# alexrenz/AdaPM

Measured on AMD Instinct MI355X. Metric: pull_push_ops_per_s, higher is better.
Workload: dtype fp32; 1 GPU; model=kge_complex_dim512, entities=10000000, relations=1000, dim=512, neg_samples=16, global_batch=16384, triples=90000000, parallelism=ps-async-dp1, fused_step=True, warmup_extra_steps=400

## Files before the change

### adapm_amd/csrc/core.cpp

```cpp
#include <torch/extension.h>
#include <ATen/Parallel.h>

#include <algorithm>
#include <atomic>
#include <condition_variable>
#include <cstring>
#include <limits>
#include <deque>
#include <map>
#include <queue>
#include <tuple>
#include <memory>
#include <mutex>
#include <random>
#include <thread>
#include <chrono>
#include <unordered_map>
#include <unordered_set>
#include <cstdio>
#include <vector>

#include "common.h"
#include "kernels.h"
#include "ops.h"
#include "ustream.h"

#ifdef ADAPM_WITH_HIP
#include <c10/hip/HIPStream.h>
#include <ATen/core/CachingHostAllocator.h>
#include <ATen/hip/impl/HIPStreamMasqueradingAsCUDA.h>
#endif

extern "C" {
int adapm_host_arena_alloc(long long floats, int want_device_visible, void** host_ptr,
                           void** dev_ptr);
void adapm_host_arena_free(void* host_ptr, int was_device_visible);
}

namespace adapm {

namespace py = pybind11;

static void* current_stream(const torch::Device& dev) {
#ifdef ADAPM_WITH_HIP
  if (dev.is_cuda()) return (void*)c10::hip::getCurrentHIPStream(dev.index()).stream();
#endif
  return nullptr;
}

static void check_step_lanes(const char* name, const char* what, int64_t lanes) {
  TORCH_CHECK(lanes <= STEP_MAX_LANES, name, ": ", what, " = ", lanes,
              " exceeds the GPU step kernels' limit of ", STEP_MAX_LANES);
}


struct Slab {
  torch::Tensor buf;
  float* data = nullptr;
  int64_t capacity = 0;
  int64_t bump = 0;
  std::unordered_map<int32_t, std::vector<int64_t>> freelists;
  std::mutex mu;
  std::atomic<int64_t> in_use{0};
  bool is_cuda = false;
  void* host_raw = nullptr;
  float* host_host = nullptr;
  float* host_dev = nullptr;
  int64_t host_capacity = 0;
  int64_t host_bump = 0;
  std::unordered_map<int32_t, std::vector<int64_t>> host_freelists;
  std::atomic<int64_t> host_in_use{0};

  static int32_t padded(int32_t len) { return (len + 3) & ~3; }

  void init(int64_t cap, const torch::Device& dev) {
    capacity = cap;
    is_cuda = dev.is_cuda();
    buf = torch::zeros({cap}, torch::TensorOptions().dtype(torch::kFloat32).device(dev));
    data = buf.data_ptr<float>();
  }

  void init_host(int64_t cap) {
    void *hp = nullptr, *dp = nullptr;
    int rc = adapm_host_arena_alloc(cap, is_cuda ? 1 : 0, &hp, &dp);
    if (rc != 0) throw std::runtime_error("host-spill arena allocation failed");
    host_raw = hp;
    host_host = (float*)hp;
    host_dev = (float*)dp;
    host_capacity = cap;
  }
  ~Slab() { adapm_host_arena_free(host_raw, is_cuda ? 1 : 0); }

  SlabBases bases() const { return SlabBases{data, is_cuda ? host_dev : host_host}; }

  int64_t try_alloc_device(int32_t len) {
    int32_t p = padded(len);
    std::lock_guard<std::mutex> g(mu);
    auto it = freelists.find(p);
    if (it != freelists.end() && !it->second.empty()) {
      int64_t off = it->second.back();
      it->second.pop_back();
      in_use += p;
      return off;
    }
    if (bump + p <= capacity) {
      int64_t off = bump;
      bump += p;
      in_use += p;
      return off;
    }
    return -1;
  }

  int64_t alloc(int32_t len) {
    int32_t p = padded(len);
    std::lock_guard<std::mutex> g(mu);
    auto it = freelists.find(p);
    if (it != freelists.end() && !it->second.empty()) {
      int64_t off = it->second.back();
      it->second.pop_back();
      in_use += p;
      return off;
    }
    if (bump + p <= capacity) {
      int64_t off = bump;
      bump += p;
      in_use += p;
      return off;
    }
    if (host_capacity > 0) {
      auto hit = host_freelists.find(p);
      if (hit != host_freelists.end() && !hit->second.empty()) {
        int64_t off = hit->second.back();
        hit->second.pop_back();
        host_in_use += p;
        return off | SPILL_BIT;
// ... 48 lines not shown
struct RespRec {
  int dest = 0;
  int64_t code = 0, key = 0, f0 = 0, f1 = 0, f2 = 0;
  int64_t slab_off = -1;
  int32_t len = 0;
  bool free_after = false;
  torch::Tensor payload;
  std::vector<Key> keys;
  std::vector<int64_t> aux;
  std::vector<int64_t> aux2;
  std::vector<int64_t> slab_offs;
};

struct IntentReq {
  int wid;
  Clock start, end;
  std::vector<Key> keys;
};

struct ChannelState {
  std::mutex mu;
  std::deque<IntentReq> intent_queue;
  std::vector<IntentReq> future_intents;
  struct IntentExpiry {
    Clock end;
    int wid;
    std::shared_ptr<std::vector<Key>> keys;
    bool operator>(const IntentExpiry& o) const { return end > o.end; }
  };
  std::priority_queue<IntentExpiry, std::vector<IntentExpiry>, std::greater<>> intent_expiry;
  std::unordered_set<Key> replicas;
  std::unordered_map<Key, uint64_t> holders;
  std::deque<OutRec> out_queue;
  std::vector<RespRec> responses;
  std::unordered_map<Key, uint32_t> reloc_ctr;
  std::unordered_map<Key, int64_t> reloc_round;
  std::atomic<int64_t> rounds{0};
  int64_t idle_streak = 0;
  std::atomic<int64_t> idle2_events{0};
};


class UniformStream {
 public:
  UniformStream(int64_t lo, int64_t hi, const std::string& device)
      : lo_(lo), hi_(hi), dev_(device) {
    TORCH_CHECK(supported(lo, hi), "UniformStream: [", lo, ", ", hi,
                ") is not a range of numpy's 32-bit bounded draw");
    excl_ = (uint32_t)((uint64_t)hi - (uint64_t)lo);
    thr_ = (uint32_t)((0x100000000ull - excl_) % excl_);
    state_ = torch::zeros({USTREAM_STATE_WORDS},
                          torch::TensorOptions().dtype(torch::kInt64).device(dev_));
  }

  static bool supported(int64_t lo, int64_t hi) {
    if (hi <= lo || lo == std::numeric_limits<int64_t>::min()) return false;
    uint64_t span = (uint64_t)hi - (uint64_t)lo;
    return span >= 2 && span <= 0xFFFFFFFFull;
  }

  void import_state(uint64_t state_hi, uint64_t state_lo, uint64_t inc_hi, uint64_t inc_lo,
                    uint64_t has_uint32, uint64_t uinteger) {
    auto h = torch::empty({USTREAM_STATE_WORDS}, torch::kInt64);
    uint64_t* p = reinterpret_cast<uint64_t*>(h.data_ptr<int64_t>());
    p[0] = state_hi, p[1] = state_lo, p[2] = inc_hi, p[3] = inc_lo;
    p[4] = has_uint32 ? 1 : 0, p[5] = uinteger & 0xFFFFFFFFull;
    ustream_build_table(p);
    std::lock_guard<std::mutex> g(mu_);
    adopt(current_stream(dev_));
    state_.copy_(h);
  }

  std::vector<uint64_t> export_state() {
    torch::Tensor h;
    {
      std::lock_guard<std::mutex> g(mu_);
      adopt(current_stream(dev_));
      h = state_.slice(0, 0, USTREAM_GEN_WORDS).cpu();
    }
    const uint64_t* p = reinterpret_cast<const uint64_t*>(h.data_ptr<int64_t>());
    return std::vector<uint64_t>(p, p + USTREAM_GEN_WORDS);
  }

  torch::Tensor draw(int64_t n, int64_t slack = -1) {
    TORCH_CHECK(n >= 0, "UniformStream.draw: n must be >= 0");
    auto opt = torch::TensorOptions().dtype(torch::kInt64).device(dev_);
    auto out = torch::empty({n}, opt);
    if (n == 0) return out;
    if (slack < 0) {
      double p = (double)thr_ / 4294967296.0;
      double w0 = (double)n / (1.0 - p);
      slack = (int64_t)std::ceil(w0 - (double)n + 8.0 * std::sqrt(w0 * p) / (1.0 - p)) + 16;
    }
    const int64_t words = n + slack;
    std::lock_guard<std::mutex> g(mu_);
    void* st = current_stream(dev_);
    adopt(st);
    auto tmp = torch::empty({ustream_tmp_words(words)}, opt);
    uint64_t* sp = reinterpret_cast<uint64_t*>(state_.data_ptr<int64_t>());
    if (dev_.is_cuda()) {
#ifdef ADAPM_WITH_HIP
      uniform_draw_gpu(sp, lo_, excl_, thr_, n, words, out.data_ptr<int64_t>(),
                       tmp.data_ptr<int64_t>(), st);
#else
      TORCH_CHECK(false, "UniformStream: built without HIP");
#endif
    } else {
      uniform_draw_cpu(sp, lo_, excl_, thr_, n, words, out.data_ptr<int64_t>(),
                       tmp.data_ptr<int64_t>());
    }
    return out;
  }

  int64_t lo() const { return lo_; }
  int64_t hi() const { return hi_; }
  const torch::Device& device() const { return dev_; }

 private:
  void adopt(void* st) {
#ifdef ADAPM_WITH_HIP
    if (dev_.is_cuda() && have_owner_ && st != owner_) hipStreamSynchronize((hipStream_t)owner_);
#endif
    owner_ = st;
    have_owner_ = true;
  }

  int64_t lo_, hi_;
  uint32_t excl_ = 0, thr_ = 0;
  torch::Device dev_;
  torch::Tensor state_;
  std::mutex mu_;
  void* owner_ = nullptr;
  bool have_owner_ = false;
};


class Server {
 public:
  Server(int64_t num_keys, torch::Tensor lens, int rank, int world, int num_channels,
         int num_workers, std::string device, double capacity_factor, int techniques,
         bool location_caches, int64_t device_cap_floats = 0, int64_t host_spill_floats = 0,
         double sync_threshold = 0.0)
      : num_keys_(num_keys),
        rank_(rank),
        world_(world),
        nch_(num_channels),
        techniques_(techniques),
        use_loc_cache_(location_caches),
        sync_threshold_(sync_threshold),
        dev_(device) {
    TORCH_CHECK((nch_ & (nch_ - 1)) == 0, "num_channels must be a power of 2");
    {
      int hw = (int)std::thread::hardware_concurrency();
      int nt = std::max(1, std::min(hw / std::max(1, world_) - 2, 31));
      if (const char* e = getenv("ADAPM_PASS_THREADS")) nt = std::max(1, atoi(e));
      pass_pool_.want_threads = nt;
    }
    log2ch_ = 0;
    while ((1 << log2ch_) < nch_) log2ch_++;

    lens = lens.to(torch::kInt32).contiguous();
    if (lens.numel() == 1) {
      uniform_len_ = lens.item<int32_t>();
    } else {
      TORCH_CHECK(lens.numel() == num_keys_, "value_lengths must have num_keys entries");
      uniform_len_ = -1;
      lens_.assign(lens.data_ptr<int32_t>(), lens.data_ptr<int32_t>() + num_keys_);
    }

    meta_ = std::vector<std::atomic<int64_t>>(num_keys_);
    version_ = std::vector<std::atomic<uint32_t>>(num_keys_);
    for (int64_t i = 0; i < num_keys_; ++i) {
      meta_[i].store(0, std::memory_order_relaxed);
      version_[i].store(0, std::memory_order_relaxed);
    }
    sync_loc_.assign(num_keys_, -1);
    if (use_loc_cache_) loc_cache_.assign(num_keys_, -1);
    int64_t n_managed = (num_keys_ + world_ - 1) / world_;
    owner_of_.assign(n_managed, rank_);
    mgr_reloc_ctr_.assign(n_managed, 0);

    int64_t owned_floats = 0;
    for (Key k = rank_; k < num_keys_; k += world_) owned_floats += Slab::padded(len_of(k));
    int64_t cap = (int64_t)((double)owned_floats * capacity_factor) + (1 << 20);
    if (device_cap_floats > 0) cap = device_cap_floats;
    slab_.init(cap, dev_);
    if (host_spill_floats > 0) {
      slab_.init_host(host_spill_floats);
      heat_.reset(new std::atomic<uint32_t>[num_keys_]);
      for (Key k = 0; k < num_keys_; ++k) heat_[k].store(0, std::memory_order_relaxed);
    }
    if (owned_floats > cap) layout_identity_.store(false);
    for (Key k = rank_; k < num_keys_; k += world_) {
      int32_t l = len_of(k);
      meta_[k] = mpack(slab_.alloc(l), F_PRESENT | F_OWNER);
    }

    intent_cnt_.reset(new std::atomic<uint16_t>[num_keys_]);
    for (Key k = 0; k < num_keys_; ++k) intent_cnt_[k].store(0, std::memory_order_relaxed);
    channels_ = std::vector<ChannelState>(nch_);
    clocks_ = std::vector<std::atomic<Clock>>(std::max(1, num_workers));
    for (auto& c : clocks_) c = 0;
    locks_ = std::make_unique<std::mutex[]>(N_STRIPES);
  }


  static constexpr int64_t MSPILL = 16;
  static constexpr int64_t MFLAGS = F_PRESENT | F_OWNER | F_STUB | F_UPDATED | F_HASREP;
  static inline int64_t mpack(int64_t loc, int64_t flags) {
    if (loc < 0) return flags;
    return ((loc & ~SPILL_BIT) << 6) | ((loc & SPILL_BIT) ? MSPILL : 0) | flags;
  }
  static inline uint8_t mflags(int64_t m) { return (uint8_t)(m & MFLAGS); }
  static inline int64_t mloc(int64_t m) {
    return (int64_t)((uint64_t)m >> 6) | ((m & MSPILL) ? SPILL_BIT : 0);
  }

  inline bool on_default_stream() const {
#ifdef ADAPM_WITH_HIP
    if (dev_.is_cuda())
      return c10::hip::getCurrentHIPStream(dev_.index()) ==
             c10::hip::getDefaultHIPStream(dev_.index());
#endif
    return true;
  }

  inline int32_t len_of(Key k) const { return uniform_len_ >= 0 ? uniform_len_ : lens_[k]; }
  inline int manager_of(Key k) const { return (int)(k % world_); }
  inline int channel_of(Key k) const {
    if (nch_ == 1) return 0;
    return (int)(((uint32_t)((uint64_t)k * 2654435769ULL)) >> (32 - log2ch_));
  }
  inline std::mutex& stripe(Key k) { return locks_[(size_t)k % N_STRIPES]; }

  int directions(Key k) {
    if (meta_[k].load(std::memory_order_acquire) & F_OWNER) return rank_;
    if (manager_of(k) == rank_) return owner_of_[k / world_];
    if (use_loc_cache_) {
      int c = loc_cache_[k];
      if (c >= 0) return c;
    }
    return manager_of(k);
  }

  struct InflightGuard {
    Server* s;
    explicit InflightGuard(Server* sv) : s(sv) {
      for (;;) {
        s->inflight_.fetch_add(1, std::memory_order_acquire);
        if (!s->migrating_.load(std::memory_order_acquire)) break;
        s->inflight_.fetch_sub(1, std::memory_order_release);
        std::this_thread::yield();
      }
    }
    ~InflightGuard() { s->inflight_.fetch_sub(1, std::memory_order_release); }
  };

  void quiesce() {
    while (inflight_.load(std::memory_order_acquire) != 0) std::this_thread::yield();
  }


  struct HostBatch {
    std::vector<int64_t> src, dst;
    std::vector<int32_t> len;
    void add(int64_t s, int64_t d, int32_t l) {
      src.push_back(s);
      dst.push_back(d);
      len.push_back(l);
    }
    size_t size() const { return src.size(); }
  };

  struct PassPool {
    struct Task {
      const std::function<void(int64_t, int64_t)>* fn = nullptr;
      int64_t n = 0;
      std::atomic<int64_t>* next = nullptr;
      std::atomic<int>* done = nullptr;
      uint64_t gen = 0;
    };
    std::vector<std::thread> threads;
    std::mutex run_mu_;
    std::mutex mu;
    std::condition_variable cv;
    Task task;
    uint64_t gen = 0;
// ... 1907 lines not shown
      if (!it->second->fail.empty()) failed_tickets_[ts] = std::move(it->second->fail);
      tickets_.erase(it);
      tickets_cv_.notify_all();
    }
  }

  void fail_ticket(int64_t ts, int cnt, const char* why) {
    std::lock_guard<std::mutex> g(tickets_mu_);
    auto it = tickets_.find(ts);
    if (it == tickets_.end()) return;
    Ticket& t = *it->second;
    t.received += cnt;
    if (t.fail.empty()) t.fail = why;
    if (t.received >= t.expected) {
      failed_tickets_[ts] = std::move(t.fail);
      tickets_.erase(it);
      tickets_cv_.notify_all();
    }
  }

  void fail(std::string reason) {
    {
      std::lock_guard<std::mutex> g(tickets_mu_);
      failed_reason_ = std::move(reason);
      failed_flag_.store(true, std::memory_order_relaxed);
      tickets_.clear();
    }
    tickets_cv_.notify_all();
    rounds_cv_.notify_all();
  }
  std::string failed_reason() {
    std::lock_guard<std::mutex> g(tickets_mu_);
    return failed_reason_;
  }

  void sync_finish(int ch, bool globally_idle = false) {
    if (globally_idle) {
      std::lock_guard<std::mutex> g(channels_[ch].mu);
      if (!channels_[ch].responses.empty()) globally_idle = false;
      for (const auto& r : channels_[ch].out_queue) {
        bool data = (r.payload.defined() && r.payload.numel() > 0) ||
                    r.code == M_PUSH_REQ || r.code == M_SET_REQ || r.code == M_PUSH_REQ_BULK;
        if (data) {
          globally_idle = false;
          break;
        }
      }
    }
    {
      std::lock_guard<std::mutex> g(rounds_mu_);
      ChannelState& C = channels_[ch];
      C.rounds++;
      if (globally_idle) {
        if (++C.idle_streak >= 2) C.idle2_events++;
      } else {
        C.idle_streak = 0;
      }
    }
    rounds_cv_.notify_all();
  }

  py::dict debug_pending() {
    py::dict d;
    {
      std::lock_guard<std::mutex> g(tickets_mu_);
      d["tickets"] = tickets_.size();
    }
    py::list outq, respq, rounds;
    for (auto& C : channels_) {
      std::lock_guard<std::mutex> g(C.mu);
      outq.append(C.out_queue.size());
      respq.append(C.responses.size());
      rounds.append(C.rounds.load());
    }
    d["out_queues"] = outq;
    d["responses"] = respq;
    d["rounds"] = rounds;
    return d;
  }


  bool fused_plain_ok(void* st) {
    if (clocks_.size() != 1 || fused_multi_stream_) return false;
    if (!fused_marks_.defined()) {
      if (getenv("ADAPM_FUSED_ATOMIC")) {
        fused_multi_stream_ = true;
        return false;
      }
      fused_marks_ = torch::zeros({rowmark_words(num_keys_)},
                                  torch::TensorOptions().dtype(torch::kInt32).device(dev_));
      if (getenv("ADAPM_FUSED_STATS"))
        fused_shared_stat_ =
            torch::zeros({1}, torch::TensorOptions().dtype(torch::kInt64).device(dev_));
      fused_marks_stream_ = st;
      return true;
    }
    if (st == fused_marks_stream_) return true;
#ifdef ADAPM_WITH_HIP
    hipStreamSynchronize((hipStream_t)fused_marks_stream_);
#endif
    fused_multi_stream_ = true;
    return false;
  }

  void check_fused_identity(const char* name, int64_t D) {
    TORCH_CHECK(world_ == 1, name, " requires a single rank (all keys local)");
    TORCH_CHECK(uniform_len_ == 2 * D, name, ": store rows must be [emb|accum] = 2D");
    TORCH_CHECK(layout_identity_.load(), name, " requires the identity layout");
    TORCH_CHECK(dev_.is_cuda(), name, " is the GPU fast path");
  }

  void count_fused_ops(int64_t keys) {
    stat_pull_keys_ += keys;
    stat_pull_local_ += keys;
    stat_push_keys_ += keys;
    stat_push_local_ += keys;
    stat_pulls_ += 1;
    stat_pushes_ += 1;
  }

  struct StagedKeys {
    torch::Tensor dev;
    std::vector<const int64_t*> ptr;
  };
  StagedKeys stage_keys(const char* name, std::initializer_list<const torch::Tensor*> parts) {
    int64_t total = 0;
    for (auto* t : parts) {
      check_keys(*t);
      total += t->numel();
    }
    auto blob = torch::empty(
        {total}, torch::TensorOptions().dtype(torch::kInt64).pinned_memory(true));
    int64_t* dst = blob.data_ptr<int64_t>();
    const uint64_t lim = (uint64_t)num_keys_;
    uint64_t bad = 0;
    for (auto* t : parts) {
      const int64_t* kp = t->data_ptr<int64_t>();
      const int64_t n = t->numel();
      for (int64_t i = 0; i < n; ++i) {
        int64_t k = kp[i];
        dst[i] = k;
        bad |= ((uint64_t)k >= lim);
      }
      dst += n;
    }
    if (bad)
      for (auto* t : parts) check_key_range(*t);
    StagedKeys sk;
    sk.dev = torch::empty({total}, torch::TensorOptions().dtype(torch::kInt64).device(dev_));
#ifdef ADAPM_WITH_HIP
    auto stream = c10::hip::getCurrentHIPStreamMasqueradingAsCUDA(dev_.index());
    TORCH_CHECK(copy_keys_gpu(sk.dev.data_ptr<int64_t>(), blob.data_ptr<int64_t>(), total,
                              (void*)stream.stream()),
                name, ": the pinned key staging buffer is not visible to the device");
    at::getHostAllocator(at::kCUDA)->record_event(
        blob.data_ptr(), blob.storage().data_ptr().get_context(), stream.unwrap());
#else
    TORCH_CHECK(false, name, ": built without HIP");
#endif
    const int64_t* dp = sk.dev.data_ptr<int64_t>();
    for (auto* t : parts) {
      sk.ptr.push_back(dp);
      dp += t->numel();
    }
    return sk;
  }

  std::tuple<torch::Tensor, torch::Tensor> kge_step_fused_impl(
      const torch::Tensor& keys_s, const torch::Tensor& keys_r, const torch::Tensor& keys_o,
      const torch::Tensor* keys_neg, UniformStream* us, int64_t N, int64_t D, double lr,
      double eps) {
    check_fused_identity("kge_step_fused", D);
    check_step_lanes("kge_step_fused", "D/2", D / 2);
    int64_t B = keys_s.numel();
    TORCH_CHECK(keys_r.numel() == B && keys_o.numel() == B);
    StagedKeys sk;
    torch::Tensor drawn;
    const int64_t* kn;
    if (us) {
      TORCH_CHECK(us->lo() >= 0 && us->hi() <= num_keys_, "kge_step_fused_sampled: stream range [",
                  us->lo(), ", ", us->hi(), ") exceeds the store's ", num_keys_, " keys");
      TORCH_CHECK(us->device() == dev_,
                  "kge_step_fused_sampled: stream is not on the store's device");
      TORCH_CHECK(N >= 0 && B * N > 0, "kge_step_fused_sampled: nothing to draw");
      sk = stage_keys("kge_step_fused", {&keys_s, &keys_r, &keys_o});
      drawn = us->draw(B * N);
      kn = drawn.data_ptr<int64_t>();
    } else {
      TORCH_CHECK(keys_neg->numel() == B * N);
      sk = stage_keys("kge_step_fused", {&keys_s, &keys_r, &keys_o, keys_neg});
      kn = sk.ptr[3];
    }
    const int64_t *ks = sk.ptr[0], *kr = sk.ptr[1], *ko = sk.ptr[2];

    auto loss = torch::empty({B}, torch::TensorOptions().dtype(torch::kFloat32).device(dev_));
    void* st = current_stream(dev_);
    {
      InflightGuard g(this);
      std::unique_lock<std::mutex> mg(fused_mu_);
      if (fused_plain_ok(st)) {
        RowMarkKeys mk{{ks, kr, ko, kn}, {B, B, B, B * N}, 4};
        auto* marks = reinterpret_cast<uint32_t*>(fused_marks_.data_ptr<int32_t>());
        rowmark_set_gpu(marks, mk, st);
        kge_complex_step_fused_gpu(
            slab_.data, mk.keys[0], mk.keys[1], mk.keys[2], mk.keys[3], loss.data_ptr<float>(),
            (int)B, (int)N, (int)D, Slab::padded(uniform_len_), world_, (float)lr, (float)eps,
            st, marks,
            fused_shared_stat_.defined()
                ? reinterpret_cast<unsigned long long*>(fused_shared_stat_.data_ptr<int64_t>())
                : nullptr);
        rowmark_clear_gpu(marks, mk, st);
        stat_fused_plain_ += 1;
      } else {
        mg.unlock();
        kge_complex_step_fused_gpu(slab_.data, ks, kr, ko, kn, loss.data_ptr<float>(), (int)B,
                                   (int)N, (int)D, Slab::padded(uniform_len_), world_, (float)lr,
                                   (float)eps, st);
        stat_fused_atomic_ += 1;
      }
    }
    count_fused_ops(3 * B + B * N);
    return {loss, drawn};
  }

  torch::Tensor kge_step_fused(torch::Tensor keys_s, torch::Tensor keys_r, torch::Tensor keys_o,
                               torch::Tensor keys_neg, int64_t N, int64_t D, double lr,
                               double eps) {
    return std::get<0>(
        kge_step_fused_impl(keys_s, keys_r, keys_o, &keys_neg, nullptr, N, D, lr, eps));
  }

  std::tuple<torch::Tensor, torch::Tensor> kge_step_fused_sampled(
      torch::Tensor keys_s, torch::Tensor keys_r, torch::Tensor keys_o, UniformStream& us,
      int64_t N, int64_t D, double lr, double eps) {
    return kge_step_fused_impl(keys_s, keys_r, keys_o, nullptr, &us, N, D, lr, eps);
  }

  struct FusedResolve {
    std::vector<std::vector<int64_t>> offs;
    std::vector<int64_t> missed;
    int64_t b_hit = 0;
    std::vector<const int64_t*> ptr;
    std::vector<torch::Tensor> dev;
  };

  FusedResolve resolve_fused(const std::vector<std::pair<const int64_t*, int>>& arrs,
                             int64_t B) {
    FusedResolve out;
    const int na = (int)arrs.size();
    constexpr int64_t G = 1024;
    int64_t nchunks = (B + G - 1) / G;
    struct Part {
      std::vector<std::vector<int64_t>> offs;
      std::vector<int64_t> missed;
    };
    std::vector<Part> parts(nchunks);
    pass_pool_.run(nchunks, [&](int64_t c0, int64_t c1) {
      for (int64_t c = c0; c < c1; ++c) {
        Part& P = parts[c];
        P.offs.resize(na);
        int64_t e = std::min(B, (c + 1) * G);
        std::vector<int64_t> tmp;
        for (int64_t b = c * G; b < e; ++b) {
          tmp.clear();
          bool ok = true;
          for (int a = 0; a < na && ok; ++a) {
            const int64_t* kp = arrs[a].first;
            int cnt = arrs[a].second;
            for (int i = 0; i < cnt; ++i) {
              Key k = kp[b * cnt + i];
              int64_t m = meta_[k].load(std::memory_order_acquire);
              uint8_t f = mflags(m);
              if (!(f & F_PRESENT) || (f & F_STUB)) { ok = false; break; }
              if (m & MSPILL) { ok = false; break; }
              tmp.push_back(mloc(m));
            }
          }
          if (!ok) {
            P.missed.push_back(b);
            continue;
          }
          size_t t = 0;
          for (int a = 0; a < na; ++a) {
            const int64_t* kp = arrs[a].first;
            int cnt = arrs[a].second;
            for (int i = 0; i < cnt; ++i) {
              Key k = kp[b * cnt + i];
              int64_t m = meta_[k].load(std::memory_order_acquire);
              if (m & F_OWNER) {
                if (m & F_HASREP) version_[k].fetch_add(1, std::memory_order_relaxed);
              } else {
                meta_[k].fetch_or((int64_t)F_UPDATED);
              }
              P.offs[a].push_back(tmp[t++]);
            }
          }
        }
      }
    });
    out.offs.resize(na);
// ... 351 lines not shown
  void enable_locality_stats() {
    locality_stats_ = true;
    key_accesses_ = std::vector<std::atomic<uint32_t>>(num_keys_);
    key_local_ = std::vector<std::atomic<uint32_t>>(num_keys_);
    for (int64_t i = 0; i < num_keys_; ++i) {
      key_accesses_[i].store(0);
      key_local_[i].store(0);
    }
  }

  void debug_set_loc_cache(int64_t k, int r) {
    TORCH_CHECK(use_loc_cache_ && (uint64_t)k < (uint64_t)num_keys_);
    loc_cache_[k] = r;
  }

  std::tuple<int, int64_t, int64_t, int> debug_key_state(int64_t k) {
    TORCH_CHECK((uint64_t)k < (uint64_t)num_keys_, "key out of range");
    int owner = -1;
    if ((Key)(k % world_) == (Key)rank_) owner = owner_of_[k / world_];
    int64_t m = meta_[k].load();
    return {(int)mflags(m), (m & F_PRESENT) ? mloc(m) : -1, (int64_t)version_[k].load(), owner};
  }

  void enable_key_trace(torch::Tensor keys) {
    std::lock_guard<std::mutex> g(trace_mu_);
    if (keys.numel() == 1 && keys.data_ptr<int64_t>()[0] == -1) {
      trace_all_ = true;
      return;
    }
    auto kc = keys.contiguous();
    for (int64_t i = 0; i < kc.numel(); ++i) traced_keys_.insert(kc.data_ptr<int64_t>()[i]);
  }

  void trace_event(Key k, const char* ev) {
    if (!trace_all_ && traced_keys_.empty()) return;
    std::lock_guard<std::mutex> g(trace_mu_);
    if (!trace_all_ && !traced_keys_.count(k)) return;
    double t = std::chrono::duration<double>(std::chrono::steady_clock::now() - t0_).count();
    trace_.push_back({t, k, ev});
  }

  void dump_locality_stats(std::string path) {
    if (!locality_stats_) return;
    FILE* f = fopen(path.c_str(), "w");
    if (!f) throw std::runtime_error("cannot open " + path);
    fprintf(f, "key\taccesses\tlocal\n");
    for (int64_t k = 0; k < num_keys_; ++k) {
      uint32_t a = key_accesses_[k].load();
      if (a) fprintf(f, "%lld\t%u\t%u\n", (long long)k, a, key_local_[k].load());
    }
    fclose(f);
  }

  void dump_traces(std::string path) {
    std::lock_guard<std::mutex> g(trace_mu_);
    FILE* f = fopen(path.c_str(), "w");
    if (!f) throw std::runtime_error("cannot open " + path);
    fprintf(f, "time_s\tkey\tevent\n");
    for (auto& e : trace_) fprintf(f, "%.6f\t%lld\t%s\n", e.t, (long long)e.k, e.ev);
    fclose(f);
  }

  py::dict stats() {
    py::dict d;
    d["pulls"] = stat_pulls_.load();
    d["pushes"] = stat_pushes_.load();
    d["pull_keys"] = stat_pull_keys_.load();
    d["push_keys"] = stat_push_keys_.load();
    d["pull_local"] = stat_pull_local_.load();
    d["push_local"] = stat_push_local_.load();
    d["pull_replica"] = stat_pull_replica_.load();
    d["push_replica"] = stat_push_replica_.load();
    d["remote_pulls_served"] = stat_remote_pulls_served_.load();
    d["remote_pushes_served"] = stat_remote_pushes_served_.load();
    d["relocations_out"] = stat_relocations_.load();
    d["relocations_in"] = stat_relocated_in_.load();
    d["replications"] = stat_replications_.load();
    d["replica_drops"] = stat_drops_.load();
    d["forwards"] = stat_forwards_.load();
    d["dropped_records"] = stat_dropped_records_.load();
    d["delta_overhops"] = stat_delta_overhops_.load();
    d["fused_plain_steps"] = stat_fused_plain_.load();
    d["fused_atomic_steps"] = stat_fused_atomic_.load();
    {
      std::lock_guard<std::mutex> g(fused_mu_);
      if (fused_shared_stat_.defined())
        d["fused_shared_occurrences"] = fused_shared_stat_.cpu().item<int64_t>();
    }
    {
      py::list hh;
      for (int i = 0; i < 9; ++i) hh.append(hop_hist_[i].load());
      d["hop_hist"] = hh;
    }
    d["replica_records"] = stat_replica_records_.load();
    d["replica_payloads"] = stat_replica_payloads_.load();
    d["bytes_sent"] = stat_bytes_sent_.load();
    d["bytes_recv"] = stat_bytes_recv_.load();
    d["sampling_checks"] = stat_sampling_checks_.load();
    d["slab_in_use"] = slab_.in_use.load();
    d["slab_capacity"] = slab_.capacity;
    d["host_spill_in_use"] = slab_.host_in_use.load();
    d["spill_rebalance_moves"] = stat_spill_moves_.load();
    d["sync_threshold"] = sync_threshold_;
    d["host_spill_capacity"] = slab_.host_capacity;
    int64_t rounds = 0;
    for (auto& c : channels_) rounds += c.rounds.load();
    d["sync_rounds"] = rounds;
    d["t_pass_ms"] = t_pass_.load() / 1e6;
    d["t_sy_intents_ms"] = t_sy_intents_.load() / 1e6;
    d["t_sy_replicas_ms"] = t_sy_replicas_.load() / 1e6;
    d["t_sy_build_ms"] = t_sy_build_.load() / 1e6;
    d["t_sy_proc_ms"] = t_sy_proc_.load() / 1e6;
    d["t_sy_apply_ms"] = t_sy_apply_.load() / 1e6;
    d["n_sy_deltas"] = n_sy_deltas_.load();
    d["n_sy_proc_recs"] = n_sy_proc_recs_.load();
    d["n_sy_apply_recs"] = n_sy_apply_recs_.load();
    d["t_todev_ms"] = t_todev_.load() / 1e6;
    d["t_launch_ms"] = t_launch_.load() / 1e6;
    d["t_misc_ms"] = t_misc_.load() / 1e6;
    d["t_calls"] = t_calls_.load();
    return d;
  }

  torch::Tensor debug_flags() {
    auto t = torch::empty({(int64_t)num_keys_}, torch::TensorOptions().dtype(torch::kUInt8));
    uint8_t* p = t.data_ptr<uint8_t>();
    for (int64_t i = 0; i < num_keys_; ++i) p[i] = mflags(meta_[i].load());
    return t;
  }

 private:
  void check_keys(const torch::Tensor& keys) {
    TORCH_CHECK(keys.device().is_cpu() && keys.scalar_type() == torch::kInt64 && keys.is_contiguous(),
                "keys must be a contiguous CPU int64 tensor");
  }

  void check_key_range(const torch::Tensor& keys) {
    const int64_t* kp = keys.data_ptr<int64_t>();
    int64_t n = keys.numel();
    uint64_t bad = 0;
    const uint64_t lim = (uint64_t)num_keys_;
    for (int64_t i = 0; i < n; ++i) bad |= ((uint64_t)kp[i] >= lim);
    if (bad) {
      for (int64_t i = 0; i < n; ++i)
        TORCH_CHECK((uint64_t)kp[i] < lim, "key out of range: ", kp[i]);
    }
  }

  void check_val_size(const torch::Tensor& keys, int64_t have, const char* op) {
    int64_t need;
    int64_t n = keys.numel();
    if (uniform_len_ >= 0) {
      need = n * (int64_t)uniform_len_;
    } else {
      need = 0;
      const int64_t* kp = keys.data_ptr<int64_t>();
      for (int64_t i = 0; i < n; ++i) {
        TORCH_CHECK((uint64_t)kp[i] < (uint64_t)num_keys_, "key out of range: ", kp[i]);
        need += lens_[kp[i]];
      }
    }
    TORCH_CHECK(have == need, op, ": value tensor has ", have, " floats but ", n,
                " key(s) need ", need);
  }

  int64_t num_keys_;
  int rank_, world_, nch_, log2ch_ = 0, techniques_;
  bool use_loc_cache_;
  torch::Device dev_;
  int32_t uniform_len_ = -1;
  std::vector<int32_t> lens_;

  Slab slab_;
  std::vector<std::atomic<int64_t>> meta_;
  std::vector<int64_t> sync_loc_;
  std::vector<std::atomic<uint32_t>> version_;
  std::vector<int32_t> loc_cache_;
  std::vector<int32_t> owner_of_;
  std::vector<uint32_t> mgr_reloc_ctr_;
  std::unique_ptr<std::mutex[]> locks_;
  std::mutex cpu_val_mu_;

  std::vector<ChannelState> channels_;
  std::unique_ptr<std::atomic<uint16_t>[]> intent_cnt_;
  std::vector<std::atomic<Clock>> clocks_;
  Clock intent_ahead_ = 1LL << 40;

  std::atomic<bool> layout_identity_{true};

  std::atomic<int> inflight_{0};
  int max_hops_ = getenv("ADAPM_MAX_HOPS") ? atoi(getenv("ADAPM_MAX_HOPS")) : 64;
  PassPool pass_pool_;
  std::atomic<int> migrating_{0};
  double sync_threshold_ = 0.0;
  std::unique_ptr<std::atomic<uint32_t>[]> heat_;
  std::mutex spill_mu_;
  std::mutex rebalance_mu_;
  std::vector<Key> spill_touched_;
  int64_t rebalance_calls_ = 0;
  std::atomic<int64_t> stat_spill_moves_{0};
  std::atomic<int64_t> next_ts_{1};
 public:
  std::atomic<int64_t> t_pass_{0}, t_todev_{0}, t_launch_{0}, t_calls_{0}, t_misc_{0};
  std::atomic<int64_t> t_sy_intents_{0}, t_sy_replicas_{0}, t_sy_build_{0}, t_sy_proc_{0},
      t_sy_apply_{0}, n_sy_deltas_{0}, n_sy_proc_recs_{0}, n_sy_apply_recs_{0};
  bool cpp_timing_ = getenv("ADAPM_CPP_TIMING") != nullptr;
 private:
  std::mutex tickets_mu_;
  std::condition_variable tickets_cv_;
  std::unordered_map<int64_t, std::unique_ptr<Ticket>> tickets_;
  std::unordered_map<int64_t, std::string> failed_tickets_;
  std::string failed_reason_;
  std::atomic<bool> failed_flag_{false};
  std::mutex rounds_mu_;
  std::condition_variable rounds_cv_;

  bool locality_stats_ = false;
  std::vector<std::atomic<uint32_t>> key_accesses_, key_local_;
  std::mutex trace_mu_;
  std::unordered_set<Key> traced_keys_;
  bool trace_all_ = false;
  struct TraceEv { double t; Key k; const char* ev; };
  std::vector<TraceEv> trace_;
  std::chrono::steady_clock::time_point t0_ = std::chrono::steady_clock::now();

  std::atomic<int64_t> hop_hist_[9] = {};
  std::atomic<int64_t> stat_replica_records_{0}, stat_replica_payloads_{0};
  std::atomic<int64_t> stat_pulls_{0}, stat_pushes_{0}, stat_pull_keys_{0}, stat_push_keys_{0},
      stat_pull_local_{0}, stat_push_local_{0}, stat_pull_replica_{0}, stat_push_replica_{0},
      stat_remote_pulls_served_{0}, stat_remote_pushes_served_{0}, stat_relocations_{0},
      stat_relocated_in_{0}, stat_replications_{0}, stat_drops_{0}, stat_forwards_{0},
      stat_dropped_records_{0}, stat_delta_overhops_{0}, stat_bytes_sent_{0},
      stat_bytes_recv_{0}, stat_sampling_checks_{0};

  std::mutex fused_mu_;
  torch::Tensor fused_marks_;
  torch::Tensor fused_shared_stat_;
  void* fused_marks_stream_ = nullptr;
  bool fused_multi_stream_ = false;
  std::atomic<int64_t> stat_fused_plain_{0}, stat_fused_atomic_{0};
};


static float* fp(torch::Tensor& t) { return t.data_ptr<float>(); }
static const float* cfp(const torch::Tensor& t) { return t.data_ptr<float>(); }

static void check_f32(const torch::Tensor& t, const char* name) {
  TORCH_CHECK(t.is_contiguous() && t.scalar_type() == torch::kFloat32, name,
              " must be contiguous float32");
}

void kge_complex_step(torch::Tensor s, torch::Tensor r, torch::Tensor o, torch::Tensor neg,
                      torch::Tensor ds, torch::Tensor dr, torch::Tensor do_, torch::Tensor dneg,
                      torch::Tensor loss, int64_t N, int64_t D, double lr, double eps) {
  for (auto* t : {&s, &r, &o, &neg, &ds, &dr, &do_, &dneg, &loss}) check_f32(*t, "kge tensor");
  int B = (int)loss.numel();
  if (s.is_cuda()) {
    TORCH_CHECK(hip_available(), "kge_complex_step: CUDA tensor but no HIP device");
    check_step_lanes("kge_complex_step", "D/2", D / 2);
    kge_complex_step_gpu(cfp(s), cfp(r), cfp(o), cfp(neg), fp(ds), fp(dr), fp(do_), fp(dneg),
                         fp(loss), B, (int)N, (int)D, (float)lr, (float)eps,
                         current_stream(s.device()));
  } else {
    kge_complex_step_cpu(cfp(s), cfp(r), cfp(o), cfp(neg), fp(ds), fp(dr), fp(do_), fp(dneg),
                         fp(loss), B, (int)N, (int)D, (float)lr, (float)eps);
  }
}

void rescal_step(torch::Tensor s, torch::Tensor r, torch::Tensor o, torch::Tensor neg,
                 torch::Tensor ds, torch::Tensor drl, torch::Tensor do_, torch::Tensor dneg,
                 torch::Tensor loss, int64_t N, int64_t D, double lr, double eps) {
  for (auto* t : {&s, &r, &o, &neg, &ds, &drl, &do_, &dneg, &loss}) check_f32(*t, "rescal");
  int B = (int)loss.numel();
  TORCH_CHECK(D <= 196, "rescal_step: dim must be <= 196 (R tile staged in LDS)");
  if (s.is_cuda()) {
    TORCH_CHECK(hip_available(), "rescal_step: CUDA tensor but no HIP device");
    rescal_step_gpu(cfp(s), cfp(r), cfp(o), cfp(neg), fp(ds), fp(drl), fp(do_), fp(dneg),
                    fp(loss), B, (int)N, (int)D, (float)lr, (float)eps,
                    current_stream(s.device()));
  } else {
    rescal_step_cpu(cfp(s), cfp(r), cfp(o), cfp(neg), fp(ds), fp(drl), fp(do_), fp(dneg),
                    fp(loss), B, (int)N, (int)D, (float)lr, (float)eps);
  }
}

void kge_complex_score(torch::Tensor s, torch::Tensor r, torch::Tensor cand,
                       torch::Tensor scores, int64_t D) {
  for (auto* t : {&s, &r, &cand, &scores}) check_f32(*t, "kge tensor");
  int B = (int)scores.size(0), E = (int)scores.size(1);
  if (s.is_cuda()) {
    TORCH_CHECK(hip_available(), "kge_complex_score: CUDA tensor but no HIP device");
    if (D % 4 == 0) {
      auto qbuf = torch::empty({(int64_t)B * D},
                               torch::TensorOptions().dtype(torch::kFloat32).device(s.device()));
      kge_complex_score_mfma_gpu(cfp(s), cfp(r), cfp(cand), fp(scores),
                                 qbuf.data_ptr<float>(), B, E, (int)D,
                                 current_stream(s.device()));
    } else {
      kge_complex_score_gpu(cfp(s), cfp(r), cfp(cand), fp(scores), B, E, (int)D,
                            current_stream(s.device()));
    }
  } else {
    kge_complex_score_cpu(cfp(s), cfp(r), cfp(cand), fp(scores), B, E, (int)D);
  }
}

torch::Tensor rescal_step_grouped(torch::Tensor s, torch::Tensor rm, torch::Tensor o,
                                  torch::Tensor neg, torch::Tensor ds, torch::Tensor drl,
                                  torch::Tensor do_, torch::Tensor dneg, torch::Tensor starts,
                                  int64_t N, int64_t D, double lr, double eps) {
  for (auto* t : {&s, &rm, &o, &neg, &ds, &drl, &do_, &dneg})
    check_f32(*t, "rescal_grouped tensor");
  TORCH_CHECK(s.is_cuda(), "rescal_step_grouped is the GPU path (CPU uses rescal_step)");
  TORCH_CHECK(D % 4 == 0, "rescal_step_grouped: D must be a multiple of 4");
  TORCH_CHECK(starts.scalar_type() == torch::kInt32 && starts.device().is_cpu() &&
              starts.is_contiguous());
  int G = (int)starts.numel() - 1;
  int B = (int)(s.numel() / (2 * D));
  TORCH_CHECK(rm.numel() == (int64_t)G * 2 * D * D, "rm must be [G][2*D*D]");
  TORCH_CHECK(starts.data_ptr<int32_t>()[G] == B, "starts[-1] must equal B");
  auto dev = s.device();
  auto opts = torch::TensorOptions().dtype(torch::kFloat32).device(dev);
  auto U = torch::empty({(int64_t)B * D}, opts);
// ... 181 lines not shown
```

Before: 1.234 billion key-ops/s.

## Overlap fused-step key staging, sampling and row marking on a prep stream

Adds a dedicated non-blocking prep stream with double-buffered row-mark arrays and events. Key staging (H2D copy), negative sampling and rowmark_set now run on that stream for step n+1 while the main stream executes step n's fused kernel. Events order the prep work after the matching mark buffer has been cleared, and the main stream waits for prep completion. The cost is a second mark array of num_keys size plus extra event and stream-sync complexity. The overlap only applies when the key count reaches a threshold.

```diff
diff --git a/adapm_amd/csrc/core.cpp b/adapm_amd/csrc/core.cpp
--- a/adapm_amd/csrc/core.cpp
+++ b/adapm_amd/csrc/core.cpp
@@ -48,10 +48,17 @@
   return nullptr;
 }
 
+struct EnqueueStream {
+  void* raw;
+  c10::Stream torch;
+};
+
 static void check_step_lanes(const char* name, const char* what, int64_t lanes) {
   TORCH_CHECK(lanes <= STEP_MAX_LANES, name, ": ", what, " = ", lanes,
               " exceeds the GPU step kernels' limit of ", STEP_MAX_LANES);
 }
+
+constexpr int64_t PREP_OVERLAP_MIN_KEYS = 131072;
 
 
 struct Slab {
@@ -266,8 +273,12 @@
     return std::vector<uint64_t>(p, p + USTREAM_GEN_WORDS);
   }
 
-  torch::Tensor draw(int64_t n, int64_t slack = -1) {
+  torch::Tensor draw(int64_t n, int64_t slack = -1) { return draw_on(n, slack, nullptr); }
+
+  torch::Tensor draw_on(int64_t n, int64_t slack, const EnqueueStream* on) {
     TORCH_CHECK(n >= 0, "UniformStream.draw: n must be >= 0");
+    c10::OptionalStreamGuard sg;
+    if (on) sg.reset_stream(on->torch);
     auto opt = torch::TensorOptions().dtype(torch::kInt64).device(dev_);
     auto out = torch::empty({n}, opt);
     if (n == 0) return out;
@@ -278,7 +289,7 @@
     }
     const int64_t words = n + slack;
     std::lock_guard<std::mutex> g(mu_);
-    void* st = current_stream(dev_);
+    void* st = on ? on->raw : current_stream(dev_);
     adopt(st);
     auto tmp = torch::empty({ustream_tmp_words(words)}, opt);
     uint64_t* sp = reinterpret_cast<uint64_t*>(state_.data_ptr<int64_t>());
@@ -387,6 +398,10 @@
     for (auto& c : clocks_) c = 0;
     locks_ = std::make_unique<std::mutex[]>(N_STRIPES);
   }
+
+  Server(const Server&) = delete;
+  Server& operator=(const Server&) = delete;
+  ~Server() { close_prep_stream(); }
 
 
   static constexpr int64_t MSPILL = 16;
@@ -2460,17 +2475,19 @@
 
   bool fused_plain_ok(void* st) {
     if (clocks_.size() != 1 || fused_multi_stream_) return false;
-    if (!fused_marks_.defined()) {
+    if (!fused_marks_[0].defined()) {
       if (getenv("ADAPM_FUSED_ATOMIC")) {
         fused_multi_stream_ = true;
         return false;
       }
-      fused_marks_ = torch::zeros({rowmark_words(num_keys_)},
-                                  torch::TensorOptions().dtype(torch::kInt32).device(dev_));
+      for (auto& m : fused_marks_)
+        m = torch::zeros({rowmark_words(num_keys_)},
+                         torch::TensorOptions().dtype(torch::kInt32).device(dev_));
       if (getenv("ADAPM_FUSED_STATS"))
         fused_shared_stat_ =
             torch::zeros({1}, torch::TensorOptions().dtype(torch::kInt64).device(dev_));
       fused_marks_stream_ = st;
+      if (!getenv("ADAPM_FUSED_SERIAL_PREP")) open_prep_stream(st);
       return true;
     }
     if (st == fused_marks_stream_) return true;
@@ -2479,6 +2496,40 @@
 #endif
     fused_multi_stream_ = true;
     return false;
+  }
+
+  void open_prep_stream(void* owner) {
+#ifdef ADAPM_WITH_HIP
+    c10::DeviceGuard dg(dev_);
+    hipStream_t p = nullptr;
+    TORCH_CHECK(hipStreamCreateWithFlags(&p, hipStreamNonBlocking) == hipSuccess,
+                "kge_step_fused: cannot create the prep stream");
+    prep_stream_ = p;
+    for (auto* ev : {&prep_done_[0], &prep_done_[1], &marks_cleared_[0], &marks_cleared_[1]}) {
+      hipEvent_t e = nullptr;
+      TORCH_CHECK(hipEventCreateWithFlags(&e, hipEventDisableTiming) == hipSuccess,
+                  "kge_step_fused: cannot create the prep events");
+      *ev = e;
+    }
+    for (void* e : marks_cleared_)
+      TORCH_CHECK(hipEventRecord((hipEvent_t)e, (hipStream_t)owner) == hipSuccess);
+    cleared_recorded_[0] = cleared_recorded_[1] = true;
+    if (const char* e = getenv("ADAPM_FUSED_PREP_MIN_KEYS")) prep_min_keys_ = atoll(e);
+#endif
+  }
+
+  void close_prep_stream() {
+#ifdef ADAPM_WITH_HIP
+    if (!prep_stream_) return;
+    (void)hipStreamSynchronize((hipStream_t)fused_marks_stream_);
+    (void)hipStreamSynchronize((hipStream_t)prep_stream_);
+    for (auto* ev : {&prep_done_[0], &prep_done_[1], &marks_cleared_[0], &marks_cleared_[1]}) {
+      if (*ev) (void)hipEventDestroy((hipEvent_t)*ev);
+      *ev = nullptr;
+    }
+    (void)hipStreamDestroy((hipStream_t)prep_stream_);
+    prep_stream_ = nullptr;
+#endif
   }
 
   void check_fused_identity(const char* name, int64_t D) {
@@ -2501,7 +2552,8 @@
     torch::Tensor dev;
     std::vector<const int64_t*> ptr;
   };
-  StagedKeys stage_keys(const char* name, std::initializer_list<const torch::Tensor*> parts) {
+  StagedKeys stage_keys(const char* name, std::initializer_list<const torch::Tensor*> parts,
+                        const EnqueueStream* on = nullptr) {
     int64_t total = 0;
     for (auto* t : parts) {
       check_keys(*t);
@@ -2525,6 +2577,8 @@
     if (bad)
       for (auto* t : parts) check_key_range(*t);
     StagedKeys sk;
+    c10::OptionalStreamGuard sg;
+    if (on) sg.reset_stream(on->torch);
     sk.dev = torch::empty({total}, torch::TensorOptions().dtype(torch::kInt64).device(dev_));
 #ifdef ADAPM_WITH_HIP
     auto stream = c10::hip::getCurrentHIPStreamMasqueradingAsCUDA(dev_.index());
@@ -2552,24 +2606,27 @@
     check_step_lanes("kge_step_fused", "D/2", D / 2);
     int64_t B = keys_s.numel();
     TORCH_CHECK(keys_r.numel() == B && keys_o.numel() == B);
-    StagedKeys sk;
-    torch::Tensor drawn;
-    const int64_t* kn;
     if (us) {
       TORCH_CHECK(us->lo() >= 0 && us->hi() <= num_keys_, "kge_step_fused_sampled: stream range [",
                   us->lo(), ", ", us->hi(), ") exceeds the store's ", num_keys_, " keys");
       TORCH_CHECK(us->device() == dev_,
                   "kge_step_fused_sampled: stream is not on the store's device");
       TORCH_CHECK(N >= 0 && B * N > 0, "kge_step_fused_sampled: nothing to draw");
-      sk = stage_keys("kge_step_fused", {&keys_s, &keys_r, &keys_o});
-      drawn = us->draw(B * N);
-      kn = drawn.data_ptr<int64_t>();
     } else {
       TORCH_CHECK(keys_neg->numel() == B * N);
-      sk = stage_keys("kge_step_fused", {&keys_s, &keys_r, &keys_o, keys_neg});
-      kn = sk.ptr[3];
-    }
-    const int64_t *ks = sk.ptr[0], *kr = sk.ptr[1], *ko = sk.ptr[2];
+    }
+
+    StagedKeys sk;
+    torch::Tensor drawn;
+    auto stage_and_draw = [&](const EnqueueStream* on) {
+      if (us) {
+        sk = stage_keys("kge_step_fused", {&keys_s, &keys_r, &keys_o}, on);
+        drawn = us->draw_on(B * N, -1, on);
+      } else {
+        sk = stage_keys("kge_step_fused", {&keys_s, &keys_r, &keys_o, keys_neg}, on);
+      }
+    };
+    auto negatives = [&]() { return us ? drawn.data_ptr<int64_t>() : sk.ptr[3]; };
 
     auto loss = torch::empty({B}, torch::TensorOptions().dtype(torch::kFloat32).device(dev_));
     void* st = current_stream(dev_);
@@ -2577,9 +2634,41 @@
       InflightGuard g(this);
       std::unique_lock<std::mutex> mg(fused_mu_);
       if (fused_plain_ok(st)) {
-        RowMarkKeys mk{{ks, kr, ko, kn}, {B, B, B, B * N}, 4};
-        auto* marks = reinterpret_cast<uint32_t*>(fused_marks_.data_ptr<int32_t>());
-        rowmark_set_gpu(marks, mk, st);
+        const int b = (int)(fused_step_no_ & 1);
+        const bool overlap = prep_stream_ != nullptr && 3 * B + B * N >= prep_min_keys_;
+#ifdef ADAPM_WITH_HIP
+        auto m_torch = c10::hip::getCurrentHIPStreamMasqueradingAsCUDA(dev_.index());
+        if (overlap) {
+          auto p_torch = c10::hip::getStreamFromExternalMasqueradingAsCUDA(
+              (hipStream_t)prep_stream_, dev_.index());
+          const EnqueueStream on{prep_stream_, p_torch.unwrap()};
+          stage_and_draw(&on);
+          if (!cleared_recorded_[b]) {
+            TORCH_CHECK(hipEventRecord((hipEvent_t)marks_cleared_[b], (hipStream_t)st) ==
+                        hipSuccess);
+            cleared_recorded_[b] = true;
+          }
+          TORCH_CHECK(hipStreamWaitEvent((hipStream_t)prep_stream_,
+                                         (hipEvent_t)marks_cleared_[b], 0) == hipSuccess);
+          sk.dev.record_stream(m_torch.unwrap());
+          if (us) drawn.record_stream(m_torch.unwrap());
+        } else {
+          stage_and_draw(nullptr);
+        }
+#else
+        stage_and_draw(nullptr);
+#endif
+        void* pre = overlap ? prep_stream_ : st;
+        RowMarkKeys mk{{sk.ptr[0], sk.ptr[1], sk.ptr[2], negatives()}, {B, B, B, B * N}, 4};
+        auto* marks = reinterpret_cast<uint32_t*>(fused_marks_[b].data_ptr<int32_t>());
+        rowmark_set_gpu(marks, mk, pre);
+#ifdef ADAPM_WITH_HIP
+        if (overlap) {
+          TORCH_CHECK(hipEventRecord((hipEvent_t)prep_done_[b], (hipStream_t)pre) == hipSuccess);
+          TORCH_CHECK(hipStreamWaitEvent((hipStream_t)st, (hipEvent_t)prep_done_[b], 0) ==
+                      hipSuccess);
+        }
+#endif
         kge_complex_step_fused_gpu(
             slab_.data, mk.keys[0], mk.keys[1], mk.keys[2], mk.keys[3], loss.data_ptr<float>(),
             (int)B, (int)N, (int)D, Slab::padded(uniform_len_), world_, (float)lr, (float)eps,
@@ -2588,12 +2677,21 @@
                 ? reinterpret_cast<unsigned long long*>(fused_shared_stat_.data_ptr<int64_t>())
                 : nullptr);
         rowmark_clear_gpu(marks, mk, st);
+#ifdef ADAPM_WITH_HIP
+        if (overlap)
+          TORCH_CHECK(hipEventRecord((hipEvent_t)marks_cleared_[b], (hipStream_t)st) ==
+                      hipSuccess);
+#endif
+        cleared_recorded_[b] = overlap;
+        fused_step_no_ += 1;
         stat_fused_plain_ += 1;
+        stat_fused_overlap_ += overlap;
       } else {
         mg.unlock();
-        kge_complex_step_fused_gpu(slab_.data, ks, kr, ko, kn, loss.data_ptr<float>(), (int)B,
-                                   (int)N, (int)D, Slab::padded(uniform_len_), world_, (float)lr,
-                                   (float)eps, st);
+        stage_and_draw(nullptr);
+        kge_complex_step_fused_gpu(slab_.data, sk.ptr[0], sk.ptr[1], sk.ptr[2], negatives(),
+                                   loss.data_ptr<float>(), (int)B, (int)N, (int)D,
+                                   Slab::padded(uniform_len_), world_, (float)lr, (float)eps, st);
         stat_fused_atomic_ += 1;
       }
     }
@@ -3111,6 +3209,7 @@
     d["delta_overhops"] = stat_delta_overhops_.load();
     d["fused_plain_steps"] = stat_fused_plain_.load();
     d["fused_atomic_steps"] = stat_fused_atomic_.load();
+    d["fused_overlap_steps"] = stat_fused_overlap_.load();
     {
       std::lock_guard<std::mutex> g(fused_mu_);
       if (fused_shared_stat_.defined())
@@ -3263,11 +3362,17 @@
       stat_bytes_recv_{0}, stat_sampling_checks_{0};
 
   std::mutex fused_mu_;
-  torch::Tensor fused_marks_;
+  torch::Tensor fused_marks_[2];
+  int64_t fused_step_no_ = 0;
   torch::Tensor fused_shared_stat_;
   void* fused_marks_stream_ = nullptr;
+  void* prep_stream_ = nullptr;
+  void* prep_done_[2] = {nullptr, nullptr};
+  void* marks_cleared_[2] = {nullptr, nullptr};
+  bool cleared_recorded_[2] = {false, false};
+  int64_t prep_min_keys_ = PREP_OVERLAP_MIN_KEYS;
   bool fused_multi_stream_ = false;
-  std::atomic<int64_t> stat_fused_plain_{0}, stat_fused_atomic_{0};
+  std::atomic<int64_t> stat_fused_plain_{0}, stat_fused_atomic_{0}, stat_fused_overlap_{0};
 };
 
 
```

Result: slower. 1.156 billion key-ops/s (-6.3%).
